# nh273/caro-ai

Hardware: AMD Instinct MI355X
Metric: self-play MCTS node-expansions/sec/GPU (Connect4, 200 sims/move); 1->8 GPU scaling (higher is better)
Workload: dtype f32

## Files before the change

caro_ai_amd/_lib.py:

```python
import ctypes as C
import os

_HERE = os.path.dirname(os.path.abspath(__file__))
LIB_PATH = os.path.join(_HERE, "libcaro_hip.so")
if os.environ.get("CARO_HIP_LIB"):
    LIB_PATH = os.environ["CARO_HIP_LIB"]

GAME_CONNECT4, GAME_MNK, GAME_CARO = 0, 1, 2
RESIGNED = -2


class CaroError(RuntimeError):
    pass


class CaroConfig(C.Structure):
    _fields_ = [
        ("game_kind", C.c_int32), ("n", C.c_int32), ("k", C.c_int32), ("n_games", C.c_int32),
        ("n_stores", C.c_int32), ("n_nets", C.c_int32), ("max_batch", C.c_int32), ("node_cap", C.c_int32),
        ("steps_before_tau_0", C.c_int32), ("first_player_mode", C.c_int32),
        ("c_puct", C.c_float), ("alpha", C.c_double), ("explore", C.c_double),
        ("seed", C.c_uint64), ("uid_base", C.c_uint64), ("uid_stride", C.c_uint64),
        ("device_id", C.c_int32), ("evict", C.c_int32), ("stagger", C.c_int32), ("stagger_recycle", C.c_int32),
        ("games_limit", C.c_int64),
# ... 81 lines not shown
    "caro_select_cancel": (C.c_int, [_P]),
    "caro_expand_backup": (C.c_int, [_P, _P, _P, _P]),
    "caro_policy": (C.c_int, [_P, _P, _P, _P]),
    "caro_step": (C.c_int, [_P, _P, _P, _P, _P, _P]),
    "caro_drain_tuples": (C.c_int, [_P, C.c_int64, _P, _P, _P, _P, _P, C.c_int, _P, _P, _P]),
    "caro_drain_tuples_begin": (C.c_int, [_P, C.c_int64, _P, _P, _P, _P, _P, C.c_int, _P]),
    "caro_drain_tuples_end": (C.c_int, [_P, _P, _P]),
    "caro_search_staggered": (C.c_int, [_P, _P, _P, C.c_int, C.c_int, _P, _P, _P, _P, _P]),
    "caro_drain_parked_begin": (C.c_int, [_P, C.c_int64, _P, _P, _P, _P, _P, _P]),
    "caro_engine_set_resign": (C.c_int, [_P, C.c_double, C.c_double]),
    "caro_drain_tuples_begin_q": (C.c_int, [_P, C.c_int64, _P, _P, _P, _P, _P, C.c_int, _P, _P]),
    "caro_drain_parked_begin_q": (C.c_int, [_P, C.c_int64, _P, _P, _P, _P, _P, _P, _P]),
    "caro_engine_set_playout_cap": (C.c_int, [_P, C.c_double, C.c_int]),
    "caro_drain_tuples_begin_x": (C.c_int, [_P, C.c_int64, _P, _P, _P, _P, _P, C.c_int, _P, _P, _P]),
    "caro_drain_parked_begin_x": (C.c_int, [_P, C.c_int64, _P, _P, _P, _P, _P, _P, _P, _P]),
    "caro_engine_set_early_stop": (C.c_int, [_P, C.c_int]),
    "caro_engine_set_openings": (C.c_int, [_P, C.c_int]),
    "caro_engine_set_forced_playouts": (C.c_int, [_P, C.c_double]),
    "caro_forced_stats": (C.c_int, [_P, _P, _P]),
    "caro_engine_set_kernel_form": (C.c_int, [_P, C.c_int]),
    "caro_engine_kernel_form": (C.c_int, [_P]),
    "caro_host_forced_root": (C.c_int, [C.c_int, _P, _P, _P, _P, C.c_double, C.c_double, _P]),
    "caro_host_forced_prune": (C.c_int, [C.c_int, _P, _P, _P, C.c_float, C.c_double, _P]),
    "caro_drain_tuples_begin_ex": (C.c_int, [_P, C.c_int64, _P, _P, _P, _P, _P, C.c_int, C.POINTER(CaroDrainExtra), _P]),
    "caro_drain_parked_begin_ex": (C.c_int, [_P, C.c_int64, _P, _P, _P, _P, _P, C.POINTER(CaroDrainExtra), _P]),
    "caro_counters": (C.c_int, [_P, _P, _P]),
    "caro_live_games": (C.c_int, [_P, _P, _P]),
    "caro_pending_leaves": (C.c_int, [_P, _P, _P]),
    "caro_debug_stamps": (C.c_int, [_P, C.c_int]),
    "caro_debug_read": (C.c_int, [_P, _P, C.c_int64, _P]),
    "caro_debug_sqrt_check": (C.c_int, [C.c_uint32, _P]),
    "caro_profile_enable": (C.c_int, [_P, C.c_int]),
    "caro_profile_read": (C.c_int, [_P, _P, _P, C.c_int]),
    "caro_profile_begin": (C.c_int, [_P, C.c_int, _P]),
    "caro_profile_end": (None, [_P, C.c_int, _P]),
    "caro_tree_sizes": (C.c_int, [_P, _P, _P]),
    "caro_tree_live": (C.c_int, [_P, _P, _P]),
    "caro_lookup_nodes": (C.c_int, [_P, C.c_int64] + [_P] * 10),
    "caro_get_roots": (C.c_int, [_P] * 6),
    "caro_poke_nodes": (C.c_int, [_P, C.c_int64] + [_P] * 9),
    "caro_backup_path": (C.c_int, [_P, C.c_int, C.c_int, C.c_float, C.c_int, C.c_int, _P, _P, _P]),
    "caro_dump_tree": (C.c_int, [_P, C.c_int, C.c_int, C.c_int64] + [_P] * 8),
}
EXPORTS = sorted(_SIGNATURES)

_lib = None


def load():
    global _lib
    if _lib is not None:
        return _lib
    if not os.path.exists(LIB_PATH):
# ... 19 lines not shown
```

caro_ai_amd/build.py:

```python
import os
import subprocess
import sys

HERE = os.path.dirname(os.path.abspath(__file__))
CSRC = os.path.join(HERE, "csrc")
OUT = os.path.join(HERE, "libcaro_hip.so")
SOURCES = [os.path.join(CSRC, "caro_engine.hip"), os.path.join(CSRC, "caro_net.hip")]
DEPS = SOURCES + [os.path.join(CSRC, "caro_rules.h"), os.path.join(CSRC, "caro_variants.h"),
                  os.path.join(CSRC, "caro_host.inc"), os.path.join(CSRC, "caro_net_kernels.inc"),
                  os.path.join(HERE, "..", "include", "caro_hip.h"),
                  os.path.join(HERE, "..", "include", "caro_noise.h")]
HIPCC = os.environ.get("HIPCC", "/opt/rocm/bin/hipcc")
FLAGS = ["--offload-arch=gfx950", "-O3", "-std=c++17", "-fPIC", "-fno-fast-math", "-Wall", "-Wno-unused-function"]
PER_FILE = {"caro_engine.hip": ["-ffp-contract=off", "-mllvm", "-disable-promote-alloca-to-lds"],
            "caro_net.hip": ["-mllvm", "-disable-promote-alloca-to-lds"]}


def stale():
    if not os.path.exists(OUT):
        return True
    t = os.path.getmtime(OUT)
    return any(os.path.getmtime(d) > t for d in DEPS)


def build(force=False, verbose=False):
    if not force and not stale():
        return OUT
    objs = []
    for src in SOURCES:
        obj = os.path.join(CSRC, os.path.basename(src) + ".o")
        cmd = [HIPCC] + FLAGS + PER_FILE[os.path.basename(src)] + ["-c", src, "-o", obj]
# ... 15 lines not shown
```

caro_ai_amd/csrc/caro_engine.hip:

```cpp
#include <hip/hip_runtime.h>

#include <cstddef>
#include <cstdio>
#include <cstdlib>
#include <cstring>
#include <string>
#include <type_traits>
#include <vector>

#include "../../include/caro_hip.h"
#include "../../include/caro_noise.h"
#include "caro_rules.h"
#include "caro_variants.h"

namespace caro {

constexpr uint32_t NSTRONG = 1u << 30;
constexpr uint32_t NMASK = NSTRONG - 1u;
constexpr int ST_DROPPED = 0, ST_TERMINAL = 1, ST_LEAF = 2;
constexpr int MAXB = 64;

enum Counter { C_SIMS, C_LEVELS, C_EXPANSIONS, C_TERMINALS, C_DROPPED, C_OVERFLOW, C_PLIES, C_FINISHED, C_N };

struct View {
// ... 33 lines not shown
  uint8_t* es_cut;
  uint16_t* es_cnt;
  uint16_t* h_mb;
  int open_n;
  int16_t* open_made;
  int16_t* pk_open;
  int fp_on;
  double fp_k;
  unsigned long long* fp_ctr;
  unsigned long long* fp_sum;
  uint4* d_rec;
  uint4* path_rec;
  uint64_t* d_key;
  int32_t* g_nleaf;
  int32_t* g_off;
  int32_t* g_tree;
  int32_t* g_class;
  int32_t* g_pack;
  int32_t* slot_list;
  int32_t* leaf_count;
  unsigned long long* counters;
  unsigned long long* counters_sum;
  unsigned long long* dbg;
  int stag_S;
  int stag_recycle;
  int stag_pool;
  int32_t* handed;
  int32_t* lm;
  int32_t* pend;
  int32_t* wait;
  int32_t* dirty;
  int32_t* pk_flag;
  int32_t* pk_ply; int32_t* pk_final_r; int32_t* pk_first; int32_t* pk_result; int32_t* pk_step;
  uint64_t* pk_uid;
  uint64_t* ph_key; int32_t* ph_player; double* ph_pi; double* ph_q; uint8_t* ph_full; uint16_t* ph_mb;
  int32_t* dr_off;
  int32_t* dr_gidx;
  int32_t* dr_sel;
  int64_t* dr_tot;
};

template <bool EXT_, bool TWO_STORES_, bool DBG_>
struct TreeOpt {
  static constexpr bool EXT = EXT_, TWO_STORES = TWO_STORES_, DBG = DBG_;
};
using TreeFull = TreeOpt<true, true, true>;
using TreeLean = TreeOpt<false, false, false>;
template <class OPT> __device__ __forceinline__ bool q_on(const View& v) { return OPT::EXT && v.q_on; }
template <class OPT> __device__ __forceinline__ bool cap_on(const View& v) { return OPT::EXT && v.cap_on; }
template <class OPT> __device__ __forceinline__ bool es_on(const View& v) { return OPT::EXT && v.es_on; }
template <class OPT> __device__ __forceinline__ bool fp_on(const View& v) { return OPT::EXT && v.fp_on; }
template <class OPT> __device__ __forceinline__ int16_t* open_made(const View& v) { return OPT::EXT ? v.open_made : nullptr; }
template <class OPT> __device__ __forceinline__ int n_stores(const View& v) { return OPT::TWO_STORES ? v.n_stores : 1; }
template <class OPT> __device__ __forceinline__ unsigned long long* dbg(const View& v) { return OPT::DBG ? v.dbg : nullptr; }

template <class R>
__device__ __forceinline__ typename R::Board load_board(const uint64_t* p) {
  typename R::Board b;
#pragma unroll
  for (int i = 0; i < R::KW; ++i) b.w[i] = p[i];
  return b;
}
template <class R>
__device__ __forceinline__ void store_board(uint64_t* p, const typename R::Board& b) {
#pragma unroll
  for (int i = 0; i < R::KW; ++i) p[i] = b.w[i];
}

__device__ __forceinline__ size_t tbase(const View& v, int t) {
  return (size_t)(t * v.ntab + (v.ntab == 2 ? v.tbl[t] : 0)) * (size_t)v.tstride;
}
__device__ __forceinline__ size_t ebase(const View& v, int t) {
  return (size_t)(t * v.etab + (v.etab == 2 ? v.tbl[t] : 0)) * (size_t)v.tstride;
}

constexpr uint64_t EMPTY_KEY = ~0ULL;

// ... 1141 lines not shown
    for (int k = 0; k < j; ++k) owner = owner && !(e_node[k] == node && e_act[k] == a);
    if (!owner) continue;
    uint32_t* row = v.edges + (eb + node) * 4 * AP;
    const uint32_t nraw = e_n[j];
    int cnt = (int)(nraw & NMASK);
    uint32_t strong = nraw & NSTRONG;
    float w = __uint_as_float(e_w[j]);
    for (int k = j; k < n; ++k) {
      if (e_node[k] == node && e_act[k] == a) {
        cnt += 1;
        w = w + e_val[k];
        if (e_strong[k]) strong = NSTRONG;
      }
    }
    row[4 * a] = (uint32_t)cnt | strong;
    row[4 * a + 1] = __float_as_uint(w);
    row[4 * a + 2] = __float_as_uint(w / (float)cnt);
  }
  CARO_XS(6)
  if (xs && lane == 0) xs[7] = (unsigned long long)total;
#undef CARO_XS
}

template <class GEO>
__global__ void k_expand_backup(View v, const float* __restrict__ probs, const float* __restrict__ values) {
  GameRegs<GEO> gr = load_game<GEO>(v, blockIdx.x);
  const int B = v.leaf_count[2], off = v.g_off[blockIdx.x];
  const ExpandPre<GEO> pre = expand_preload<GEO, false>(v, blockIdx.x, B, off, probs, values);
  expand_body<GEO>(v, gr, B, pre, off, probs);
}

template <class GEO>
__device__ __forceinline__ void noise_wave(const View& v, int B, int go, uint64_t uid, uint32_t ply, int mb,
                                           double* s_nz, volatile int* s_flag) {
  constexpr int LPD = GEO::LPD, APL = GEO::APL, AP = GEO::AP;
  const int lane = threadIdx.x & 63;
  const int b = lane / LPD, l = lane % LPD;
  if (go) {
    double nz[APL];
    const uint64_t key = caro_noise_key(v.seed, uid, ply, (uint32_t)(mb * B + b));
    __shared__ double s_mail[APL > 1 ? 2 * AP : 1];
    noise_group<LPD, APL>(key, l, v.A, v.alpha, nz, s_mail);
#pragma unroll
    for (int j = 0; j < APL; ++j) s_nz[b * AP + l * APL + j] = nz[j];
  }
  __builtin_amdgcn_fence(__ATOMIC_RELEASE, "workgroup");
// ... 9 lines not shown
  __shared__ double s_nz[MAXB * 0 + 64 * GEO::APL];
  __shared__ int s_flag;
  if (threadIdx.x == 0) s_flag = 0;
  __syncthreads();
  if (threadIdx.x >= 64) {
    const int g = blockIdx.x;
    const int go = do_select && !noise && !v.done[g] && !(cap_on<OPT>(v) && mb_index >= v.cap_fast && v.fast[g]) &&
                   !(es_on<OPT>(v) && mb_index > 0 && v.es_cut[g]);
    noise_wave<GEO>(v, B, go, go ? v.uid[g] : 0ull, go ? (uint32_t)v.ply[g] : 0u, mb_index, s_nz, &s_flag);
    return;
  }
  __builtin_amdgcn_s_setprio(3);
  if (blockIdx.x == 0 && threadIdx.x == 0) {
    rows_next[0] = 0;
    rows_next[1] = 0;
    rows_next[2] = B;
    rows_cur[2] = B;
  }
  unsigned long long t0 = 0;
  if (dbg<OPT>(v)) t0 = __builtin_amdgcn_s_memtime();
  GameRegs<GEO> gr = load_game<GEO, OPT>(v, blockIdx.x);
  const ExpandPre<GEO> pre = expand_preload<GEO, true>(v, blockIdx.x, B, blockIdx.x * B, probs, values);
  if (do_expand) {
    expand_body<GEO, true, OPT>(v, gr, B, pre, blockIdx.x * B, probs);
    block_sync<true>();
  }
  const unsigned long long t1 = dbg<OPT>(v) ? __builtin_amdgcn_s_memtime() : 0;
  if (dbg<OPT>(v) && threadIdx.x == 0 && !do_select) dbg<OPT>(v)[(size_t)blockIdx.x * 8 + 5] = t1 - t0;
  if (do_select) select_body<GEO, true, OPT>(v, gr, B, mb_index, noise, rows_cur, planes, leaf_keys, s_nz, &s_flag);
  if (dbg<OPT>(v) && threadIdx.x == 0 && do_select) {
    dbg<OPT>(v)[(size_t)blockIdx.x * 8 + 6] = t1 - t0;
    dbg<OPT>(v)[(size_t)blockIdx.x * 8 + 7] = __builtin_amdgcn_s_memtime() - t0;
  }
}

template <class GEO>
__device__ __forceinline__ void root_policy(const View& v, int g, int t, const typename GEO::R::Board& root,
                                            double* s_pi, int* s_n) {
  using R = typename GEO::R;
  constexpr int AP = GEO::AP;
  const int node = probe<R>(v, t, root);
  for (int a = threadIdx.x; a < AP; a += blockDim.x)
    s_n[a] = (node >= 0 && a < v.A) ? (int)(v.edges[((ebase(v, t) + node) * AP + a) * 4] & NMASK) : 0;
  __syncthreads();
  __shared__ int s_best;
  __shared__ double s_total;
  if (threadIdx.x == 0) {
// ... 610 lines not shown
    rows_next[1] = 0;
    rows_next[2] = B;
    rows_cur[2] = B;
  }
  const unsigned long long t0 = dbg<OPT>(v) ? __builtin_amdgcn_s_memtime() : 0;
  if (w > 0) {
    if (threadIdx.x == 0) {
      v.wait[g] = w - 1;
      v.g_nleaf[g] = 0;
      v.g_class[g] = 0;
      v.g_pack[g] = 0;
    }
    return;
  }
  if (gr.done == 2) {
    if (threadIdx.x == 0) {
      v.g_nleaf[g] = 0;
      v.g_class[g] = 0;
      v.g_pack[g] = 0;
    }
    return;
  }
  if (pend) {
    expand_body<GEO, true, OPT>(v, gr, B, pre, g * B, probs);
    block_sync<true>();
  }
  const unsigned long long t1 = dbg<OPT>(v) ? __builtin_amdgcn_s_memtime() : 0;
  int over = gr.done == 1;
  if (!over && (lm >= due || cut)) {
    over = step_body<GEO, true, OPT>(v, g, gr, nullptr, s_pi, s_n, nullptr, nullptr, nullptr);
    lm = 0;
  }
  if (over) {
    if (park_and_restart<GEO, true, OPT>(v, g, gr)) over = 0;
  }
  const unsigned long long t2 = dbg<OPT>(v) ? __builtin_amdgcn_s_memtime() : 0;
  select_body<GEO, true, OPT>(v, gr, B, lm, nullptr, rows_cur, planes, leaf_keys, s_nz, &s_flag);
  if (threadIdx.x == 0) {
    v.lm[g] = over ? 0 : lm + 1;
    v.pend[g] = over ? 0 : 1;
    if (dbg<OPT>(v)) {
      dbg<OPT>(v)[(size_t)g * 8 + 5] = ((t2 - t1) & 0xFFFFFFull) | (__builtin_amdgcn_s_memrealtime() << 24);
      dbg<OPT>(v)[(size_t)g * 8 + 6] = t1 - t0;
      dbg<OPT>(v)[(size_t)g * 8 + 7] = __builtin_amdgcn_s_memtime() - t0;
      dbg<OPT>(v)[(size_t)g * 8 + 4] |= (unsigned long long)__builtin_amdgcn_s_getreg((31 << 11) | 4) << 8;
    }
  }
// ... 560 lines not shown
struct caro_engine {
  caro_config cfg;
  Variant var;
  View v;
  std::vector<void*> allocs;
  int32_t* pinned;
  int64_t* pinned64;
  int32_t* scratch;
  int32_t* live;
  int select_pending;
  int drain_pending;
  int ls_mid;
  int ls_forced;
  int stag_batch;
  hipEvent_t drain_ev;
  int prof_on;
  int prof_gate;
  uint64_t prof_ctr;
  uint64_t prof_cal;
  int32_t* rows;
  int rows_par;
  int fused_ok;
  int force_full;
  std::vector<hipEvent_t> ev;
  std::vector<int> ev_kind;
  size_t ev_used;
  double prof_ms[8];
  long long prof_n[8];
};

static bool tree_lean(const caro_engine* h) {
  const View& v = h->v;
  return !h->force_full && !v.q_on && !v.cap_on && !v.es_on && !v.open_made && !v.fp_on && v.n_stores == 1 && !v.dbg;
}

constexpr unsigned PROF_EVERY = 23;
enum ProfKind { PK_SELECT = 0, PK_COMPACT = 1, PK_EXPAND = 2, PK_STEP = 3, PK_NET = 4, PK_NULL1 = 5, PK_NULL2 = 6, PK_N = 8 };
__global__ void k_prof_null() {}
static void prof_calibrate(caro_engine* h, hipStream_t st);

static void prof_flush(caro_engine* h) {
  for (size_t i = 0; i < h->ev_used; ++i) {
    float ms = 0.f;
    if (hipEventSynchronize(h->ev[2 * i + 1]) == hipSuccess &&
        hipEventElapsedTime(&ms, h->ev[2 * i], h->ev[2 * i + 1]) == hipSuccess) {
      h->prof_ms[h->ev_kind[i]] += ms;
      h->prof_n[h->ev_kind[i]] += 1;
    }
  }
  h->ev_used = 0;
}
static int prof_begin(caro_engine* h, int kind, hipStream_t st) {
  if (!h->prof_on || !h->prof_gate) return -1;
  if (h->ev_used * 2 + 2 > h->ev.size()) {
    if (h->ev.size() >= 2 * 16384) prof_flush(h);
    else
// ... 17 lines not shown
  const int a = prof_begin(h, PK_NULL1, st);
  hipLaunchKernelGGL(k_prof_null, dim3(1), dim3(64), 0, st);
  prof_end(h, a, st);
  const int b = prof_begin(h, PK_NULL2, st);
  hipLaunchKernelGGL(k_prof_null, dim3(1), dim3(64), 0, st);
  hipLaunchKernelGGL(k_prof_null, dim3(1), dim3(64), 0, st);
  prof_end(h, b, st);
}

template <class T>
static int dalloc(caro_engine* h, T** p, size_t n) {
  void* q = nullptr;
  hipError_t e = hipMalloc(&q, n * sizeof(T) + 256);
  if (e != hipSuccess) return fail(CARO_E_NOMEM, std::string("hipMalloc failed: ") + hipGetErrorString(e));
  h->allocs.push_back(q);
  *p = (T*)q;
  return 0;
}

extern "C" {

const char* caro_last_error(void) { return g_err.c_str(); }
void caro__set_error(const char* msg) { g_err = msg ? msg : ""; }
int caro_version(void) { return 104; }

#include "caro_host.inc"

int caro_rules_move_batch(int kind, int n, int k, int64_t M, uint64_t* keys, const int32_t* moves,
                          const int32_t* players, int32_t* won, int32_t* full, void* stream) {
  const Variant var = pick_variant(kind, n);
  const GameParams gp = make_gp(kind, n, k);
  if (M <= 0) return 0;
  const unsigned grid = (unsigned)((M + 255) / 256);
  DISPATCH(var, hipLaunchKernelGGL(k_rules_move<GEO>, dim3(grid), dim3(256), 0, (hipStream_t)stream, gp,
                                   (long long)M, keys, moves, players, won, full));
  HIPCHK(hipGetLastError());
  return 0;
}
int caro_rules_legal_batch(int kind, int n, int k, int64_t M, const uint64_t* keys, uint8_t* legal, void* stream) {
  const Variant var = pick_variant(kind, n);
  const GameParams gp = make_gp(kind, n, k);
  if (M <= 0) return 0;
  const unsigned grid = (unsigned)((M * gp.A + 255) / 256);
  DISPATCH(var, hipLaunchKernelGGL(k_rules_legal<GEO>, dim3(grid), dim3(256), 0, (hipStream_t)stream, gp,
                                   (long long)M, keys, legal));
  HIPCHK(hipGetLastError());
  return 0;
// ... 101 lines not shown
  if (cfg->device_id < 0 || cfg->device_id >= ndev) return fail(CARO_E_INVAL, "device_id out of range");
  HIPCHK(hipSetDevice(cfg->device_id));

  caro_engine* h = new caro_engine();
  h->cfg = *cfg;
  h->var = var;
  h->select_pending = 0;
  h->ls_mid = 0;
  h->ls_forced = 0;
  h->prof_on = 0;
  h->prof_gate = 1;
  h->prof_ctr = 0;
  h->prof_cal = 0;
  h->rows = nullptr;
  h->rows_par = 0;
  {
    const char* e = getenv("CARO_NO_FUSED_TREE");
    h->fused_ok = !(e && e[0] == '1');
  }
  h->ev_used = 0;
  for (int i = 0; i < 8; ++i) { h->prof_ms[i] = 0; h->prof_n[i] = 0; }
  View& v = h->v;
  memset(&v, 0, sizeof v);
  v.gp = make_gp(cfg->game_kind, cfg->n, cfg->k);
  v.G = cfg->n_games;
  v.n_stores = cfg->n_stores;
  v.n_nets = cfg->n_nets;
  v.A = v.gp.A;
  v.HW = v.gp.rows * v.gp.cols;
  v.maxply = v.HW;
  v.maxd = v.HW;
  v.maxB = cfg->max_batch;
  v.ntab = (cfg->evict || cfg->stagger > 0) ? 2 : 1;
  v.etab = cfg->evict ? 2 : 1;
  apply_run_params(h, cfg);
  v.cap = cfg->node_cap > 0 ? cfg->node_cap : 4096;
  static_assert(MAXB <= 255, "leaf rank travels in 8 bits of d_rec.x");
  if (v.cap > (1 << 23)) { delete h; return fail(CARO_E_INVAL, "node_cap too large: at most 2^23 nodes per tree (slot ids travel in 24 bits)"); }
  int hc = 64;
  while (hc < 2 * v.cap) hc <<= 1;
  v.hcap = hc;
  if (v.A > 256 || v.maxd > 255) { delete h; return fail(CARO_E_INVAL, "board too large for the path records (actions < 256, depth <= 255)"); }
  {
    const char* e = getenv("CARO_TREE_SKEW");
    const long skew = e ? strtol(e, nullptr, 0) : 0;
    if (skew < 0 || skew > 65536) { delete h; return fail(CARO_E_INVAL, "CARO_TREE_SKEW must be 0 .. 65536 slots"); }
// ... 630 lines not shown
  if (!h) return fail(CARO_E_INVAL, "null engine");
  if (form != 0 && form != 1) return fail(CARO_E_INVAL, "kernel form must be 0 (automatic) or 1 (always the full form)");
  h->force_full = form;
  return 0;
}
int caro_engine_kernel_form(const caro_engine* h) {
  if (!h) return fail(CARO_E_INVAL, "null engine");
  return tree_lean(h) ? 0 : 1;
}

int caro_debug_stamps(caro_engine* h, int on) {
  if (!h) return fail(CARO_E_INVAL, "null engine");
  if (on && !h->v.dbg) {
    void* q = nullptr;
    HIPCHK(hipMalloc(&q, (size_t)h->v.G * 16 * sizeof(unsigned long long)));
    HIPCHK(hipMemset(q, 0, (size_t)h->v.G * 16 * sizeof(unsigned long long)));
    h->allocs.push_back(q);
    h->v.dbg = (unsigned long long*)q;
  } else if (!on) {
    h->v.dbg = nullptr;
  }
  return 0;
}
int caro_debug_read(caro_engine* h, uint64_t* out_host, int64_t n_u64, void* stream) {
  if (!h || !out_host || !h->v.dbg) return fail(CARO_E_INVAL, "no stamp buffer");
  if (n_u64 > (int64_t)h->v.G * 16) n_u64 = (int64_t)h->v.G * 16;
  HIPCHK(hipStreamSynchronize((hipStream_t)stream));
  HIPCHK(hipMemcpy(out_host, h->v.dbg, n_u64 * sizeof(uint64_t), hipMemcpyDeviceToHost));
  return 0;
}

int caro_debug_sqrt_check(uint32_t n_max, uint64_t* bad_host) {
  if (!bad_host || n_max > (1u << 24)) return fail(CARO_E_INVAL, "bad argument");
  unsigned long long* bad = nullptr;
  HIPCHK(hipMalloc(&bad, sizeof(unsigned long long)));
  HIPCHK(hipMemset(bad, 0, sizeof(unsigned long long)));
  hipLaunchKernelGGL(k_sqrt_check, dim3(1024), dim3(256), 0, (hipStream_t) nullptr, n_max, bad);
  HIPCHK(hipGetLastError());
  HIPCHK(hipMemcpy(bad_host, bad, sizeof(unsigned long long), hipMemcpyDeviceToHost));
  HIPCHK(hipFree(bad));
  return 0;
}

int caro_select_cancel(caro_engine* h) {
  if (!h) return fail(CARO_E_INVAL, "null engine");
  h->select_pending = 0;
// ... 141 lines not shown
```

caro_ai_amd/csrc/caro_host.inc:

```
int caro_key_words(int kind, int n) { return variant_kw(pick_variant(kind, n)); }
int caro_action_space(int kind, int n) { return kind == CARO_GAME_CONNECT4 ? 7 : n * n; }
int caro_obs_cells(int kind, int n) { return kind == CARO_GAME_CONNECT4 ? 42 : n * n; }

#define HOST_DISPATCH(var, EXPR) DISPATCH(var, EXPR)

int caro_host_initial(int kind, int n, int k, uint64_t* key) {
  const Variant var = pick_variant(kind, n);
  const GameParams gp = make_gp(kind, n, k);
  HOST_DISPATCH(var, { auto b = GEO::R::initial(gp); for (int i = 0; i < GEO::KW; ++i) key[i] = b.w[i]; });
  return 0;
}
int caro_host_move(int kind, int n, int k, uint64_t* key, int move, int player, int* won) {
  const Variant var = pick_variant(kind, n);
  const GameParams gp = make_gp(kind, n, k);
  if (player != 0 && player != 1) return fail(CARO_E_INVAL, "player must be 0 or 1");
  if (move < 0 || move >= gp.A) return fail(CARO_E_INVAL, "move out of range");
  HOST_DISPATCH(var, {
    typename GEO::R::Board b;
    for (int i = 0; i < GEO::KW; ++i) b.w[i] = key[i];
    if (kind == CARO_GAME_CONNECT4 && !GEO::R::legal(gp, b, move)) return fail(CARO_E_INVAL, "column is full");
    *won = GEO::R::move(gp, b, move, player) ? 1 : 0;
    for (int i = 0; i < GEO::KW; ++i) key[i] = b.w[i];
  });
  return 0;
// ... 78 lines not shown
  }
  return count;
}
int caro_host_forced_prune(int A, const int32_t* N, const double* Q, const float* P, float c_puct, double k,
                           int32_t* N_out) {
  if (A < 1 || A > 256) return fail(CARO_E_INVAL, "A out of range");
  if (!N || !Q || !P || !N_out) return fail(CARO_E_INVAL, "null argument");
  if (int rc = forced_k_check(k, "caro_host_forced_prune")) return rc;
  long long T = 0;
  int b = 0;
  for (int a = 0; a < A; ++a) {
    if (N[a] < 0 || N[a] >= (1 << 30)) return fail(CARO_E_INVAL, "visit count out of range");
    if (N[a] > N[b]) b = a;
    T += N[a];
  }
  if (T >= (1ll << 30)) return fail(CARO_E_INVAL, "visit total out of range");
  if (T == 0) return fail(CARO_E_INVAL, "caro_host_forced_prune: a row without visits has no policy (a refused ply)");
  const double sq = caro_sqrt((double)T), c = (double)c_puct;
  const double sstar = fp_score(Q[b], c, (double)P[b], sq, N[b]);
  for (int a = 0; a < A; ++a)
    N_out[a] = (a == b || N[a] == 0) ? N[a] : fp_pruned(N[a], Q[a], (double)P[a], c, k, (int)T, sq, sstar);
  return b;
}
```

caro_ai_amd/csrc/caro_variants.h:

```cpp
#ifndef CARO_VARIANTS_H
#define CARO_VARIANTS_H

#include "../../include/caro_noise.h"

namespace caro {

template <class R_, int LPD_, int APL_>
struct Geo {
  using R = R_;
  static constexpr int LPD = LPD_, APL = APL_, AP = LPD_ * APL_, KW = R_::KW;
};
using GeoC4 = Geo<C4Rules, 8, 1>;
using GeoM16 = Geo<MnkRules<1>, 16, 1>;
using GeoM32 = Geo<MnkRules<1>, 32, 1>;
using GeoM64 = Geo<MnkRules<1>, 64, 1>;
using GeoM128 = Geo<MnkRules<2>, 64, 2>;
using GeoM256 = Geo<MnkRules<4>, 64, 4>;
using GeoK16 = Geo<CaroRules<1>, 16, 1>;
using GeoK32 = Geo<CaroRules<1>, 32, 1>;
using GeoK64 = Geo<CaroRules<1>, 64, 1>;
using GeoK128 = Geo<CaroRules<2>, 64, 2>;
using GeoK256 = Geo<CaroRules<4>, 64, 4>;

enum Variant { V_C4, V_M16, V_M32, V_M64, V_M128, V_M256, V_K16, V_K32, V_K64, V_K128, V_K256, V_BAD };

static inline Variant pick_variant(int kind, int n) {
// ... 116 lines not shown
```

include/caro_hip.h:

```cpp
#ifndef CARO_HIP_H
#define CARO_HIP_H

#include <stdint.h>

#ifdef __cplusplus
extern "C" {
#endif

#define CARO_GAME_CONNECT4 0
#define CARO_GAME_MNK 1
#define CARO_GAME_CARO 2

#define CARO_E_INVAL (-22)
#define CARO_E_NOMEM (-12)
#define CARO_E_HIP (-5)
#define CARO_E_NODEV (-19)
#define CARO_E_STATE (-71)

#define CARO_RESIGNED (-2)

typedef struct caro_engine caro_engine;

typedef struct caro_config {
  int32_t game_kind;
// ... 21 lines not shown
int caro_version(void);

int caro_key_words(int game_kind, int n);
int caro_action_space(int game_kind, int n);
int caro_obs_cells(int game_kind, int n);

int caro_host_initial(int game_kind, int n, int k, uint64_t* key);
int caro_host_move(int game_kind, int n, int k, uint64_t* key, int move, int player, int* won);
int caro_host_legal(int game_kind, int n, int k, const uint64_t* key, uint8_t* legal);
int caro_host_encode(int game_kind, int n, int k, const uint64_t* key, int who_move, float* planes);
int caro_host_noise_row(uint64_t seed, uint64_t uid, uint32_t ply, uint32_t sim, int A, double alpha, double* out);
double caro_host_move_uniform(uint64_t seed, uint64_t uid, uint32_t ply);
double caro_host_resign_uniform(uint64_t seed, uint64_t uid);
double caro_host_cap_uniform(uint64_t seed, uint64_t uid, uint32_t ply);
double caro_host_open_uniform(uint64_t seed, uint64_t uid, uint32_t i);
int caro_host_opening(int game_kind, int n, int k, uint64_t seed, uint64_t uid, int first, int max_plies,
                      uint64_t* key_out, int* player_out, int* made_out);

int caro_host_forced_root(int A, const int32_t* N, const float* P, const double* noise, const uint8_t* legal,
                          double explore, double k, uint8_t* forced_out);
int caro_host_forced_prune(int A, const int32_t* N, const double* Q, const float* P, float c_puct, double k,
                           int32_t* N_out);

int caro_rules_move_batch(int game_kind, int n, int k, int64_t M, uint64_t* keys_dev, const int32_t* moves_dev,
                          const int32_t* players_dev, int32_t* won_dev, int32_t* full_dev, void* stream);
int caro_rules_legal_batch(int game_kind, int n, int k, int64_t M, const uint64_t* keys_dev, uint8_t* legal_dev,
                           void* stream);
int caro_rules_encode_batch(int game_kind, int n, int k, int64_t M, const uint64_t* keys_dev,
                            const int32_t* who_dev, float* planes_dev, void* stream);
int caro_noise_batch(uint64_t seed, int64_t M, int A, double alpha, const uint64_t* uid_dev, const uint32_t* ply_dev,
                     const uint32_t* sim_dev, double* out_dev, void* stream);

int caro_openings_batch(int game_kind, int n, int k, uint64_t seed, int max_plies, int64_t M, const uint64_t* uid_dev,
                        const int32_t* first_dev, uint64_t* keys_dev, int32_t* players_dev, int32_t* made_dev,
                        void* stream);

int caro_engine_create(const caro_config* cfg, caro_engine** out);
void caro_engine_destroy(caro_engine* h);
int caro_engine_restart(caro_engine* h, const caro_config* cfg, void* stream);
int caro_reset_games(caro_engine* h, const int32_t* first_player_dev, void* stream);
int caro_set_roots(caro_engine* h, const uint64_t* keys_dev, const int32_t* players_dev, void* stream);

int caro_select(caro_engine* h, int batch, int mb_index, const double* noise_dev, float* planes_dev,
                uint64_t* leaf_keys_dev, void* stream);
int caro_get_descent(caro_engine* h, int game, int b, int32_t* info_dev, float* value_dev, uint64_t* leaf_key_dev,
                     uint64_t* path_keys_dev, int32_t* path_actions_dev, void* stream);
// ... 35 lines not shown
int caro_engine_set_kernel_form(caro_engine* h, int form);
int caro_engine_kernel_form(const caro_engine* h);

typedef struct caro_drain_extra {
  uint32_t size;
  double* root_q_dev;
  uint8_t* full_dev;
  uint16_t* minibatches_dev;
  int16_t* open_dev;
} caro_drain_extra;
int caro_drain_tuples_begin_ex(caro_engine* h, int64_t cap, uint64_t* states_dev, int32_t* players_dev, double* pi_dev,
                               int32_t* z_dev, int64_t* games_dev, int recycle, const caro_drain_extra* extra,
                               void* stream);
int caro_drain_parked_begin_ex(caro_engine* h, int64_t cap, uint64_t* states_dev, int32_t* players_dev, double* pi_dev,
                               int32_t* z_dev, int64_t* games_dev, const caro_drain_extra* extra, void* stream);

int caro_counters(caro_engine* h, int64_t counters[8], void* stream);
int caro_profile_enable(caro_engine* h, int on);
int caro_profile_begin(caro_engine* h, int kind, void* stream);
void caro_profile_end(caro_engine* h, int slot, void* stream);
int caro_profile_read(caro_engine* h, double ms[8], int64_t launches[8], int reset);
int caro_debug_stamps(caro_engine* h, int on);
int caro_debug_read(caro_engine* h, uint64_t* out_host, int64_t n_u64, void* stream);
int caro_debug_sqrt_check(uint32_t n_max, uint64_t* bad_host);
int caro_live_games(caro_engine* h, int32_t* live, void* stream);
int caro_pending_leaves(caro_engine* h, int32_t* pending, void* stream);

int caro_tree_sizes(caro_engine* h, int32_t* out_dev, void* stream);
int caro_tree_live(caro_engine* h, int32_t* out_dev, void* stream);
int caro_lookup_nodes(caro_engine* h, int64_t M, const int32_t* game_dev, const int32_t* store_dev,
                      const uint64_t* keys_dev, int32_t* found_dev, int32_t* N_dev, float* W_dev, float* Q_dev,
                      float* P_dev, int32_t* strong_dev, void* stream);
int caro_get_roots(caro_engine* h, uint64_t* keys_dev, int32_t* players_dev, int32_t* ply_dev, uint64_t* uid_dev,
                   void* stream);
int caro_poke_nodes(caro_engine* h, int64_t M, const int32_t* game_dev, const int32_t* store_dev,
                    const uint64_t* keys_dev, const int32_t* N_dev, const float* W_dev, const float* Q_dev,
                    const float* P_dev, const int32_t* strong_dev, void* stream);
int caro_backup_path(caro_engine* h, int game, int store, float value, int value_is_f32, int len,
                     const uint64_t* keys_dev, const int32_t* actions_dev, void* stream);
int caro_dump_tree(caro_engine* h, int game, int store, int64_t cap, uint64_t* keys_dev, int32_t* N_dev,
                   float* W_dev, float* Q_dev, float* P_dev, int32_t* strong_dev, int64_t* n_nodes, void* stream);

typedef struct caro_net caro_net;
int64_t caro_net_packed_size(int H, int W, int A);
int caro_net_create(int H, int W, int A, float negative_slope, const float* packed_host, int64_t n_floats,
                    int device_id, caro_net** out);
// ... 59 lines not shown
```

Before: 8.540 million.

## Replace serial per-descent backup with wave-parallel grouped edge backup in expand

Result: no change. 8.601 million, median of 6 (+0.7%).

```diff
diff --git a/caro_ai_amd/_lib.py b/caro_ai_amd/_lib.py
--- a/caro_ai_amd/_lib.py
+++ b/caro_ai_amd/_lib.py
@@ -127,6 +127,7 @@
     "caro_engine_kernel_form": (C.c_int, [_P]),
     "caro_host_forced_root": (C.c_int, [C.c_int, _P, _P, _P, _P, C.c_double, C.c_double, _P]),
     "caro_host_forced_prune": (C.c_int, [C.c_int, _P, _P, _P, C.c_float, C.c_double, _P]),
+    "caro_host_backup_order": (C.c_int, [C.c_int] + [_P] * 7),
     "caro_drain_tuples_begin_ex": (C.c_int, [_P, C.c_int64, _P, _P, _P, _P, _P, C.c_int, C.POINTER(CaroDrainExtra), _P]),
     "caro_drain_parked_begin_ex": (C.c_int, [_P, C.c_int64, _P, _P, _P, _P, _P, C.POINTER(CaroDrainExtra), _P]),
     "caro_counters": (C.c_int, [_P, _P, _P]),
@@ -134,6 +135,7 @@
     "caro_pending_leaves": (C.c_int, [_P, _P, _P]),
     "caro_debug_stamps": (C.c_int, [_P, C.c_int]),
     "caro_debug_read": (C.c_int, [_P, _P, C.c_int64, _P]),
+    "caro_debug_backup_levels": (C.c_int, [_P, C.c_int]),
     "caro_debug_sqrt_check": (C.c_int, [C.c_uint32, _P]),
     "caro_profile_enable": (C.c_int, [_P, C.c_int]),
     "caro_profile_read": (C.c_int, [_P, _P, _P, C.c_int]),
diff --git a/caro_ai_amd/build.py b/caro_ai_amd/build.py
--- a/caro_ai_amd/build.py
+++ b/caro_ai_amd/build.py
@@ -7,6 +7,7 @@
 OUT = os.path.join(HERE, "libcaro_hip.so")
 SOURCES = [os.path.join(CSRC, "caro_engine.hip"), os.path.join(CSRC, "caro_net.hip")]
 DEPS = SOURCES + [os.path.join(CSRC, "caro_rules.h"), os.path.join(CSRC, "caro_variants.h"),
+                  os.path.join(CSRC, "caro_backup.h"),
                   os.path.join(CSRC, "caro_host.inc"), os.path.join(CSRC, "caro_net_kernels.inc"),
                   os.path.join(HERE, "..", "include", "caro_hip.h"),
                   os.path.join(HERE, "..", "include", "caro_noise.h")]
diff --git a/caro_ai_amd/csrc/caro_backup.h b/caro_ai_amd/csrc/caro_backup.h
--- /dev/null
+++ b/caro_ai_amd/csrc/caro_backup.h
@@ -0,0 +1,42 @@
+#ifndef CARO_BACKUP_H
+#define CARO_BACKUP_H
+
+#include <stdint.h>
+
+namespace caro {
+
+constexpr int BK_LEVELS = 16;
+
+CR_HD int bk_popc(uint64_t m) {
+  int n = 0;
+  for (; m; m &= m - 1ull) ++n;
+  return n;
+}
+CR_HD int bk_lowest(uint64_t m) {
+  int i = 0;
+  while (!((m >> i) & 1ull)) ++i;
+  return i;
+}
+
+CR_HD int bk_qpos(uint64_t m_term, uint64_t m_leaf, int b) {
+  const uint64_t below = (1ull << b) - 1ull;
+  if ((m_term >> b) & 1ull) return bk_popc(m_term & below);
+  if ((m_leaf >> b) & 1ull) return bk_popc(m_term) + bk_popc(m_leaf & below);
+  return -1;
+}
+template <class F>
+CR_HD void bk_for_each(uint64_t m_term, uint64_t m_leaf, F&& f) {
+#if defined(__HIP_DEVICE_COMPILE__)
+  for (uint64_t m = m_term; m; m &= m - 1ull) f(__builtin_ctzll(m), false);
+  for (uint64_t m = m_leaf; m; m &= m - 1ull) f(__builtin_ctzll(m), true);
+#else
+  for (uint64_t m = m_term; m; m &= m - 1ull) f(bk_lowest(m), false);
+  for (uint64_t m = m_leaf; m; m &= m - 1ull) f(bk_lowest(m), true);
+#endif
+}
+CR_HD int bk_level(int len, int r) { return len - 1 - r; }
+CR_HD float bk_addend(float value, int len, int level) { return (bk_level(len, level) & 1) ? value : -value; }
+
+}
+
+#endif
diff --git a/caro_ai_amd/csrc/caro_engine.hip b/caro_ai_amd/csrc/caro_engine.hip
--- a/caro_ai_amd/csrc/caro_engine.hip
+++ b/caro_ai_amd/csrc/caro_engine.hip
@@ -79,6 +79,7 @@
   unsigned long long* counters;
   unsigned long long* counters_sum;
   unsigned long long* dbg;
+  int bk_levels;
   int stag_S;
   int stag_recycle;
   int stag_pool;
@@ -110,6 +111,7 @@
 template <class OPT> __device__ __forceinline__ int16_t* open_made(const View& v) { return OPT::EXT ? v.open_made : nullptr; }
 template <class OPT> __device__ __forceinline__ int n_stores(const View& v) { return OPT::TWO_STORES ? v.n_stores : 1; }
 template <class OPT> __device__ __forceinline__ unsigned long long* dbg(const View& v) { return OPT::DBG ? v.dbg : nullptr; }
+template <class OPT> __device__ __forceinline__ int bk_levels(const View& v) { return OPT::DBG ? v.bk_levels : BK_LEVELS; }
 
 template <class R>
 __device__ __forceinline__ typename R::Board load_board(const uint64_t* p) {
@@ -1297,6 +1299,216 @@
 #undef CARO_XS
 }
 
+template <int AP>
+__device__ __forceinline__ void backup_path_rec_at(const View& v, size_t eb, float value, bool strong_val, const uint4* rec,
+                                                   int len) {
+  float cur = -value;
+  for (int i = len - 1; i >= 0; --i) {
+    const uint32_t na = rec[i].x;
+    uint32_t* row = v.edges + (eb + (na & 0xFFFFFFu)) * 4 * AP;
+    const int a = (int)(na >> 24);
+    const uint32_t nraw = row[4 * a];
+    const int n = (int)(nraw & NMASK) + 1;
+    const uint32_t strong = (nraw & NSTRONG) | (strong_val ? NSTRONG : 0u);
+    const float w = __uint_as_float(row[4 * a + 1]) + cur;
+    row[4 * a] = (uint32_t)n | strong;
+    row[4 * a + 1] = __float_as_uint(w);
+    row[4 * a + 2] = __float_as_uint(w / (float)n);
+    cur = -cur;
+  }
+}
+__device__ __forceinline__ float readlane_f(float x, int l) {
+  return __uint_as_float((uint32_t)__builtin_amdgcn_readlane((int)__float_as_uint(x), l));
+}
+
+template <class GEO, class OPT>
+__device__ __forceinline__ void expand_regs(const View& v, GameRegs<GEO>& gr, int B, const ExpandPre<GEO>& pre, int off) {
+  using R = typename GEO::R;
+  using Board = typename R::Board;
+  constexpr int AP = GEO::AP, KW = GEO::KW, LPD = GEO::LPD;
+  __shared__ uint64_t s_brd[8][KW];
+  __shared__ int s_node[8];
+  const int g = blockIdx.x;
+  if (gr.done) return;
+  const int lane = threadIdx.x;
+  unsigned long long* xs = dbg<OPT>(v) ? dbg<OPT>(v) + ((size_t)v.G + g) * 8 : nullptr;
+#define CARO_XS(n) if (xs && lane == 0) xs[n] = __builtin_amdgcn_s_memtime();
+  CARO_XS(0)
+  asm volatile("" ::"v"(pre.p0.x), "v"(pre.p0.y), "v"(pre.p0.z), "v"(pre.p1.x), "v"(pre.p1.y), "v"(pre.p1.z),
+               "v"(pre.row_val), "v"(pre.rec.x));
+#pragma unroll
+  for (int k = 0; k < ExpandPre<GEO>::NPR; ++k) asm volatile("" ::"v"(pre.pr[k]));
+  const int st_sel = n_stores<OPT>(v) == 2 ? gr.player : 0;
+  const int t = g * n_stores<OPT>(v) + st_sel;
+  const int nleaf = pre.nleaf;
+  const int base = st_sel ? gr.nn[1] : gr.nn[0];
+  const bool overflow = base + nleaf > v.cap;
+  const int A = v.A;
+  const int tsel = st_sel ? gr.tbl[1] : gr.tbl[0];
+  const size_t tb = tbase_sel(v, t, tsel);
+  const size_t eb = ebase_sel(v, t, tsel);
+  const int my_st = (int)(pre.rec.x & 0xFFu), my_len = (int)((pre.rec.x >> 8) & 0xFFu);
+  const int my_local = (int)((pre.rec.x >> 16) & 0xFFu);
+  const uint32_t my_home = pre.rec.z;
+  const Board& brd = pre.brd;
+  const bool is_term = lane < B && my_st == ST_TERMINAL;
+  const bool is_leaf = lane < B && my_st == ST_LEAF && !overflow;
+  const float row_val = __shfl(pre.row_val, my_local, 64);
+  const float my_val = is_leaf ? row_val : __uint_as_float(pre.rec.y);
+  CARO_XS(1)
+  int my_node = -2;
+  if (!overflow) {
+    bool clash = false;
+#pragma unroll
+    for (int bb = 0; bb < 64 / LPD; ++bb) {
+      const int ob = __builtin_amdgcn_readlane((int)is_leaf, bb);
+      const uint32_t oh = (uint32_t)__builtin_amdgcn_readlane((int)(my_home & 0x7fffffffu), bb);
+      clash = clash || (bb < lane && ob && oh == (my_home & 0x7fffffffu));
+    }
+    const bool fast = is_leaf && (my_home >> 31) != 0u && !clash;
+    if (fast) {
+      uint64_t* k = v.node_key + (tb + (my_home & 0x7fffffffu)) * KW;
+#pragma unroll
+      for (int w = KW - 1; w >= 0; --w) k[w] = brd.w[w];
+      my_node = (int)(my_home & 0x7fffffffu);
+    }
+    const bool late = is_leaf && !fast;
+    const unsigned long long slow = __ballot(late);
+    if (slow) {
+      if (late) {
+#pragma unroll
+        for (int w = 0; w < KW; ++w) s_brd[lane][w] = brd.w[w];
+      }
+      block_sync<true>();
+      if (lane == 0)
+        for (unsigned long long m = slow; m; m &= m - 1ull) {
+          const int b = __ffsll(m) - 1;
+          Board lb;
+#pragma unroll
+          for (int w = 0; w < KW; ++w) lb.w[w] = s_brd[b][w];
+          s_node[b] = insert_key<R>(v, t, lb);
+        }
+      block_sync<true>();
+      if (late) my_node = s_node[lane];
+    }
+    if (lane == 0) {
+      unsigned long long* ctr = v.counters + (size_t)g * C_N;
+      v.n_nodes[t] = base + nleaf;
+      atomicAdd(v.n_created + t, nleaf);
+      atomicAdd(ctr + C_EXPANSIONS, (unsigned long long)nleaf);
+    }
+    if (st_sel) gr.nn[1] = base + nleaf;
+    else gr.nn[0] = base + nleaf;
+  } else if (lane == 0) {
+    atomicAdd(v.counters + (size_t)g * C_N + C_OVERFLOW, 1ull);
+  }
+  CARO_XS(2)
+  const unsigned long long m_term = __ballot(is_term);
+  const unsigned long long m_leaf = __ballot(is_leaf);
+  const bool seq = overflow || __ballot((is_term || is_leaf) && my_len > bk_levels<OPT>(v)) != 0ull;
+  CARO_XS(3)
+  CARO_XS(4)
+  if (!overflow) {
+    const int b = LPD >= 64 ? 0 : lane / LPD;
+    const int nr = __shfl(my_node >= 0 ? my_node | (my_local << 24) : -1, b, 64);
+    const int node = nr >= 0 ? nr & 0xFFFFFF : -2, rank = nr >= 0 ? nr >> 24 : 0;
+#pragma unroll
+    for (int kk = 0; kk < ExpandPre<GEO>::NPR; ++kk) {
+      const int a = lane + 64 * kk - b * AP;
+      const int src = node >= 0 ? rank * AP + a : lane;
+      float pv = 0.f;
+#pragma unroll
+      for (int k = 0; k < ExpandPre<GEO>::NPR; ++k) {
+        const float x = __shfl(pre.pr[k], src & 63, 64);
+        pv = (src >> 6) == k ? x : pv;
+      }
+      if (node >= 0) {
+        uint32_t* row = v.edges + (eb + node) * 4 * AP;
+        if (a >= A) pv = 0.f;
+        reinterpret_cast<uint4*>(row)[a] = make_uint4(0u, 0u, 0u, __float_as_uint(pv));
+      }
+    }
+  }
+  CARO_XS(5)
+  int total = 0;
+  if (xs) bk_for_each(m_term, m_leaf, [&](int d, bool) { total += __builtin_amdgcn_readlane(my_len, d); });
+  if (seq) {
+    bk_for_each(m_term, m_leaf, [&](int d, bool strong_d) {
+      const float val = readlane_f(my_val, d);
+      const int len = __builtin_amdgcn_readlane(my_len, d);
+      if (lane == 0)
+        backup_path_rec_at<AP>(v, eb, val, strong_d, v.path_rec + ((size_t)g * v.maxB + d) * v.maxd, len);
+    });
+    CARO_XS(6)
+    if (xs && lane == 0) xs[7] = (unsigned long long)total;
+    return;
+  }
+  const int db = lane >> 3, lv = lane & 7;
+  const int dlen = __shfl(my_len, db, 64);
+  const bool dq = (((m_term | m_leaf) >> db) & 1ull) != 0ull;
+  const bool v0 = dq && lv < dlen, v1 = dq && 8 + lv < dlen;
+  const int key0 = (int)pre.p0.x, key1 = (int)pre.p1.x;
+  unsigned long long todo0 = __ballot(v0), todo1 = __ballot(v1);
+  const bool deep = todo1 != 0ull;
+  bool own0 = false, own1 = false;
+  unsigned long long g0m0 = 0ull, g0m1 = 0ull, g1m1 = 0ull;
+  while (todo0) {
+    const int lead = __ffsll((unsigned long long)todo0) - 1;
+    const int k = __builtin_amdgcn_readlane(key0, lead);
+    const unsigned long long m0 = __ballot(v0 && key0 == k);
+    const unsigned long long m1 = deep ? __ballot(v1 && key1 == k) : 0ull;
+    if (lane == lead) { own0 = true; g0m0 = m0; g0m1 = m1; }
+    todo0 &= ~m0;
+    todo1 &= ~m1;
+  }
+  while (todo1) {
+    const int lead = __ffsll((unsigned long long)todo1) - 1;
+    const int k = __builtin_amdgcn_readlane(key1, lead);
+    const unsigned long long m1 = __ballot(v1 && key1 == k);
+    if (lane == lead) { own1 = true; g1m1 = m1; }
+    todo1 &= ~m1;
+  }
+  int cnt0 = (int)(pre.p0.y & NMASK), cnt1 = (int)(pre.p1.y & NMASK);
+  uint32_t strong0 = pre.p0.y & NSTRONG, strong1 = pre.p1.y & NSTRONG;
+  float w0 = __uint_as_float(pre.p0.z), w1 = __uint_as_float(pre.p1.z);
+  bk_for_each(m_term, m_leaf, [&](int d, bool strong_d) {
+    const float val = readlane_f(my_val, d);
+    const int len = __builtin_amdgcn_readlane(my_len, d);
+    const uint32_t h0 = (uint32_t)(g0m0 >> (8 * d)) & 0xFFu, h1 = (uint32_t)(g0m1 >> (8 * d)) & 0xFFu;
+    if (h0 | h1) {
+      const int level = h0 ? __ffs((int)h0) - 1 : 8 + __ffs((int)h1) - 1;
+      cnt0 += 1;
+      w0 = w0 + bk_addend(val, len, level);
+      if (strong_d) strong0 = NSTRONG;
+    }
+    if (deep) {
+      const uint32_t h = (uint32_t)(g1m1 >> (8 * d)) & 0xFFu;
+      if (h) {
+        cnt1 += 1;
+        w1 = w1 + bk_addend(val, len, 8 + __ffs((int)h) - 1);
+        if (strong_d) strong1 = NSTRONG;
+      }
+    }
+  });
+  if (own0) {
+    uint32_t* row = v.edges + (eb + ((uint32_t)key0 & 0xFFFFFFu)) * 4 * AP;
+    const int a = (int)((uint32_t)key0 >> 24);
+    row[4 * a] = (uint32_t)cnt0 | strong0;
+    row[4 * a + 1] = __float_as_uint(w0);
+    row[4 * a + 2] = __float_as_uint(w0 / (float)cnt0);
+  }
+  if (own1) {
+    uint32_t* row = v.edges + (eb + ((uint32_t)key1 & 0xFFFFFFu)) * 4 * AP;
+    const int a = (int)((uint32_t)key1 >> 24);
+    row[4 * a] = (uint32_t)cnt1 | strong1;
+    row[4 * a + 1] = __float_as_uint(w1);
+    row[4 * a + 2] = __float_as_uint(w1 / (float)cnt1);
+  }
+  CARO_XS(6)
+  if (xs && lane == 0) xs[7] = (unsigned long long)total;
+#undef CARO_XS
+}
+
 template <class GEO>
 __global__ void k_expand_backup(View v, const float* __restrict__ probs, const float* __restrict__ values) {
   GameRegs<GEO> gr = load_game<GEO>(v, blockIdx.x);
@@ -1352,7 +1564,7 @@
   GameRegs<GEO> gr = load_game<GEO, OPT>(v, blockIdx.x);
   const ExpandPre<GEO> pre = expand_preload<GEO, true>(v, blockIdx.x, B, blockIdx.x * B, probs, values);
   if (do_expand) {
-    expand_body<GEO, true, OPT>(v, gr, B, pre, blockIdx.x * B, probs);
+    expand_regs<GEO, OPT>(v, gr, B, pre, blockIdx.x * B);
     block_sync<true>();
   }
   const unsigned long long t1 = dbg<OPT>(v) ? __builtin_amdgcn_s_memtime() : 0;
@@ -2009,7 +2221,7 @@
     return;
   }
   if (pend) {
-    expand_body<GEO, true, OPT>(v, gr, B, pre, g * B, probs);
+    expand_regs<GEO, OPT>(v, gr, B, pre, g * B);
     block_sync<true>();
   }
   const unsigned long long t1 = dbg<OPT>(v) ? __builtin_amdgcn_s_memtime() : 0;
@@ -2616,6 +2828,7 @@
   int rows_par;
   int fused_ok;
   int force_full;
+  int bk_debug;
   std::vector<hipEvent_t> ev;
   std::vector<int> ev_kind;
   size_t ev_used;
@@ -2625,7 +2838,7 @@
 
 static bool tree_lean(const caro_engine* h) {
   const View& v = h->v;
-  return !h->force_full && !v.q_on && !v.cap_on && !v.es_on && !v.open_made && !v.fp_on && v.n_stores == 1 && !v.dbg;
+  return !h->force_full && !h->bk_debug && !v.q_on && !v.cap_on && !v.es_on && !v.open_made && !v.fp_on && v.n_stores == 1 && !v.dbg;
 }
 
 constexpr unsigned PROF_EVERY = 23;
@@ -2689,7 +2902,7 @@
 
 const char* caro_last_error(void) { return g_err.c_str(); }
 void caro__set_error(const char* msg) { g_err = msg ? msg : ""; }
-int caro_version(void) { return 104; }
+int caro_version(void) { return 105; }
 
 #include "caro_host.inc"
 
@@ -2837,6 +3050,7 @@
   for (int i = 0; i < 8; ++i) { h->prof_ms[i] = 0; h->prof_n[i] = 0; }
   View& v = h->v;
   memset(&v, 0, sizeof v);
+  v.bk_levels = BK_LEVELS;
   v.gp = make_gp(cfg->game_kind, cfg->n, cfg->k);
   v.G = cfg->n_games;
   v.n_stores = cfg->n_stores;
@@ -3513,6 +3727,13 @@
   }
   return 0;
 }
+int caro_debug_backup_levels(caro_engine* h, int n) {
+  if (!h) return fail(CARO_E_INVAL, "null engine");
+  if (n < 0 || n > BK_LEVELS) return fail(CARO_E_INVAL, "backup levels must be in [0, 16]");
+  h->v.bk_levels = n;
+  h->bk_debug = 1;
+  return 0;
+}
 int caro_debug_read(caro_engine* h, uint64_t* out_host, int64_t n_u64, void* stream) {
   if (!h || !out_host || !h->v.dbg) return fail(CARO_E_INVAL, "no stamp buffer");
   if (n_u64 > (int64_t)h->v.G * 16) n_u64 = (int64_t)h->v.G * 16;
diff --git a/caro_ai_amd/csrc/caro_host.inc b/caro_ai_amd/csrc/caro_host.inc
--- a/caro_ai_amd/csrc/caro_host.inc
+++ b/caro_ai_amd/csrc/caro_host.inc
@@ -124,3 +124,28 @@
     N_out[a] = (a == b || N[a] == 0) ? N[a] : fp_pruned(N[a], Q[a], (double)P[a], c, k, (int)T, sq, sstar);
   return b;
 }
+
+int caro_host_backup_order(int B, const uint8_t* status, const int32_t* len, const int32_t* edges, int32_t* qpos_out,
+                           int32_t* edge_out, int32_t* descent_out, int32_t* sign_out) {
+  if (B < 1 || B > 8) return fail(CARO_E_INVAL, "caro_host_backup_order: B must be in [1, 8]");
+  if (!status || !len || !edges || !qpos_out || !edge_out || !descent_out || !sign_out)
+    return fail(CARO_E_INVAL, "null argument");
+  uint64_t m_term = 0, m_leaf = 0;
+  for (int b = 0; b < B; ++b) {
+    if (status[b] > 2) return fail(CARO_E_INVAL, "caro_host_backup_order: status must be 0, 1 or 2");
+    if (len[b] < 1 || len[b] > BK_LEVELS) return fail(CARO_E_INVAL, "caro_host_backup_order: len must be in [1, 16]");
+    if (status[b] == 1) m_term |= 1ull << b;
+    if (status[b] == 2) m_leaf |= 1ull << b;
+  }
+  for (int b = 0; b < B; ++b) qpos_out[b] = bk_qpos(m_term, m_leaf, b);
+  int n = 0;
+  bk_for_each(m_term, m_leaf, [&](int d, bool) {
+    for (int level = 0; level < len[d]; ++level) {
+      edge_out[n] = edges[d * BK_LEVELS + level];
+      descent_out[n] = d;
+      sign_out[n] = bk_addend(1.0f, len[d], level) > 0.f ? 1 : -1;
+      ++n;
+    }
+  });
+  return n;
+}
diff --git a/caro_ai_amd/csrc/caro_variants.h b/caro_ai_amd/csrc/caro_variants.h
--- a/caro_ai_amd/csrc/caro_variants.h
+++ b/caro_ai_amd/csrc/caro_variants.h
@@ -2,6 +2,7 @@
 #define CARO_VARIANTS_H
 
 #include "../../include/caro_noise.h"
+#include "caro_backup.h"
 
 namespace caro {
 
diff --git a/include/caro_hip.h b/include/caro_hip.h
--- a/include/caro_hip.h
+++ b/include/caro_hip.h
@@ -67,6 +67,9 @@
 int caro_host_forced_prune(int A, const int32_t* N, const double* Q, const float* P, float c_puct, double k,
                            int32_t* N_out);
 
+int caro_host_backup_order(int B, const uint8_t* status, const int32_t* len, const int32_t* edges, int32_t* qpos_out,
+                           int32_t* edge_out, int32_t* descent_out, int32_t* sign_out);
+
 int caro_rules_move_batch(int game_kind, int n, int k, int64_t M, uint64_t* keys_dev, const int32_t* moves_dev,
                           const int32_t* players_dev, int32_t* won_dev, int32_t* full_dev, void* stream);
 int caro_rules_legal_batch(int game_kind, int n, int k, int64_t M, const uint64_t* keys_dev, uint8_t* legal_dev,
@@ -148,6 +151,7 @@
 int caro_profile_read(caro_engine* h, double ms[8], int64_t launches[8], int reset);
 int caro_debug_stamps(caro_engine* h, int on);
 int caro_debug_read(caro_engine* h, uint64_t* out_host, int64_t n_u64, void* stream);
+int caro_debug_backup_levels(caro_engine* h, int n);
 int caro_debug_sqrt_check(uint32_t n_max, uint64_t* bad_host);
 int caro_live_games(caro_engine* h, int32_t* live, void* stream);
 int caro_pending_leaves(caro_engine* h, int32_t* pending, void* stream);
```
